# belacks/audio-denoising

Hardware: AMD Instinct MI355X
Metric: denoised audio frames/sec (32 ms, 16 kHz, hop 512) at batch 256; 1/2/4/8 GPU (higher is better)
Workload: dtype f32; 1 GPU; configs[1]: batch 256 synthetic 32 ms frames per GPU, n_fft=1024 hop=512 n_mels=80, GRUUNet2 fp32 (dari_tult weights, num_compressed_bins=5), 32-iter Griffin-Lim, device-RNG initial phases, hx carried; a step = one hop of 256 resident synthetic frames per GPU (the hops of a group are different frames; the same buffers are re-processed step after step: the path is compute-bound, no data-dependent w; streams_per_gpu=256, hops_per_launch=4, n_fft=1024, hop=512, n_mels=80, griffinlim_iters=32, conv_precision=fp32, parallelism=stream-sharded x1 (no data-path collective)

## Files before the change

audio-denoising_amd/csrc/dn_api.hip:

```cpp
#include <math.h>
#include <stdlib.h>
#include <string.h>

#include <atomic>
#include <thread>
#include <map>
#include <mutex>
#include <string>
#include <vector>

#include "dn_internal.hpp"

namespace {

thread_local std::string g_err;

int fail(int code, const std::string& msg) {
    g_err = msg;
    return code;
}

#define DN_HIP(call)                                                                                     \
    do {                                                                                                 \
        hipError_t e_ = (call);                                                                          \
// ... 853 lines not shown

size_t dn_clip_workspace_bytes(const dn_dsp* d, int32_t B, int32_t N) {
    if (!d || B <= 0 || N <= 0 || d->cfg.n_mels <= 0 || (long long)B * N > kClipMaxFrames) return 0;
    const size_t frames = (size_t)B * (size_t)N;
    return ((frames * (clip_row_floats(d) + 6 * (size_t)d->cfg.n_mels + 1) * sizeof(float) + 255) & ~size_t(255)) + 256;
}

size_t dn_clip_workspace_bytes_ex(const dn_dsp* d, int32_t B, int32_t N, uint32_t flags) {
    if (flags & ~(uint32_t)(DN_CONV_BF16 | DN_PHASE_FROM_INPUT | DN_CLIP_GL_PER_COLUMN | DN_CLIP_GL_PER_STREAM)) return 0;
    const size_t base = dn_clip_workspace_bytes(d, B, N);
    return base == 0 || !(flags & DN_PHASE_FROM_INPUT) ? base : base + phasor_bytes(d, (size_t)B * (size_t)N);
}

int dn_clip_process(const dn_model* m, const dn_dsp* d, const void* hops_in, int32_t in_s16, float* ring, float* ola, float* hx, void* hops_out,
                    int32_t out_s16, const float* init_angles, uint64_t seed, uint64_t stream_id0, int32_t n_iter, float momentum,
                    void* workspace, int32_t B, int32_t N, uint32_t flags, void* stream) {
    if (B < 1 || N < 1) return fail(DN_ERR_INVALID, "dn_clip_process: needs B >= 1 streams and N >= 1 hops");
    if (!hops_in || !ring || !ola || !hx || !hops_out || !workspace) return fail(DN_ERR_INVALID, "dn_clip_process: null argument");
    const uint32_t gl = flags & (uint32_t)(DN_CLIP_GL_PER_COLUMN | DN_CLIP_GL_PER_STREAM);
    int rc = check_hop_args("dn_clip_process", m, d, B, n_iter, momentum, flags & ~gl);
    if (rc != DN_OK) return rc;
    if (gl == (uint32_t)(DN_CLIP_GL_PER_COLUMN | DN_CLIP_GL_PER_STREAM))
        return fail(DN_ERR_INVALID, "dn_clip_process: DN_CLIP_GL_PER_COLUMN and DN_CLIP_GL_PER_STREAM exclude each other");
    if ((gl & DN_CLIP_GL_PER_STREAM) && d->cfg.n_fft != 1024)
        return fail(DN_ERR_UNSUPPORTED, "the wavefront-per-stream Griffin-Lim is built for n_fft 1024 (at 1536 the per-lane state of a stream does not fit a wavefront's registers; at 512 the schedule is not built)");
    if ((flags & DN_PHASE_FROM_INPUT) && init_angles) return fail(DN_ERR_INVALID, "dn_clip_process: DN_PHASE_FROM_INPUT takes the phases from the input: init_angles must be NULL");
    if ((long long)B * N > kClipMaxFrames)
        return fail(DN_ERR_INVALID, "dn_clip_process: B x N exceeds " + std::to_string(kClipMaxFrames) + " frames a call (tile the clip)");
    const int M = d->cfg.n_mels, C = M / 16;
    BiasSet* bs = nullptr;
    rc = build_bias(const_cast<dn_model*>(m), C, &bs);
    if (rc != DN_OK) return rc;
    dn::ClipArgs a{};
    a.hops_in = hops_in; a.in_s16 = in_s16 != 0; a.ring = ring; a.ola = ola; a.hx = hx; a.hops_out = hops_out; a.out_s16 = out_s16 != 0;
    a.init = init_angles; a.seed = seed; a.sid0 = stream_id0; a.n_iter = n_iter; a.mom = momentum / (1.0f + momentum);
    a.C = C; a.B = B; a.N = N; a.n_fft = d->cfg.n_fft; a.n_mels = M;
    a.frames = (size_t)B * (size_t)N;
    a.fr = static_cast<float*>(workspace); a.fr_stride = clip_row_floats(d);
    a.mel = a.fr + a.frames * a.fr_stride; a.diff = a.mel + a.frames * 3 * M; a.peak = a.diff + a.frames * 3 * M;
    if (flags & DN_PHASE_FROM_INPUT) a.phas = reinterpret_cast<float*>(static_cast<char*>(workspace) + dn_clip_workspace_bytes(d, B, N));
    a.per_stream = d->cfg.n_fft == 1024 && ((gl & DN_CLIP_GL_PER_STREAM) || (gl == 0 && (long)a.frames >= dn::kClipGlwAutoFrames));
    dn::launch_clip(d->view, bs->view_dev, a, (flags & DN_CONV_BF16) != 0, as_stream(stream));
    return check_launch("dn_clip_process");
}

static size_t slot_floats(const dn_dsp* d, int32_t B) {
    return (size_t)B * (6 * (size_t)d->cfg.n_mels + 1 + dn::kSlotMeta + 3 * ((size_t)d->cfg.n_fft / 2 + 1));
}

static int default_head_start(const dn_pipe* p) {
    return p->depth == 1 && p->B <= 256 ? (p->d->cfg.n_fft == 1536 ? 12 : 8) : 0;
}

int dn_pipe_create(const dn_model* m, const dn_dsp* d, int32_t B, uint32_t flags, dn_pipe** out) {
    if (!out) return fail(DN_ERR_INVALID, "dn_pipe_create: null argument");
    if (B <= 0) return fail(DN_ERR_INVALID, "dn_pipe_create: batch must be positive");
    int rc = check_hop_args("dn_pipe_create", m, d, B, 0, 0.0f, flags);
    if (rc != DN_OK) return rc;
    dn_pipe* p = new dn_pipe();
    p->m = const_cast<dn_model*>(m); p->d = const_cast<dn_dsp*>(d); p->B = B; p->C = d->cfg.n_mels / 16;
    p->bf16 = (flags & DN_CONV_BF16) != 0;
    p->phase_in = (flags & DN_PHASE_FROM_INPUT) != 0;
    p->m->refs.fetch_add(1);
    p->d->refs.fetch_add(1);
    rc = build_bias(p->m, p->C, &p->bs);
    if (rc != DN_OK) { dn_pipe_destroy(p); return rc; }
    p->slot_floats = (slot_floats(d, B) + 63) & ~size_t(63);
    p->init_elems = (size_t)B * 3 * (d->cfg.n_fft / 2 + 1);
    p->state_elems = (size_t)B * 3 * (2 * ((size_t)d->cfg.n_fft / 128) + 2) * 64;
    static_assert(sizeof(dn::PipeCtl) <= 256, "the control block fits its allocation");
    hipError_t e = hipMalloc(reinterpret_cast<void**>(&p->ctl), 256);
    if (e == hipSuccess) e = hipMemset(p->ctl, 0, 256);
    if (e == hipSuccess) e = hipMalloc(reinterpret_cast<void**>(&p->scratch), p->n_slots * p->slot_floats * sizeof(float));
    if (e == hipSuccess && p->phase_in) e = hipMalloc(reinterpret_cast<void**>(&p->scratch_init), p->n_slots * p->init_elems * sizeof(float2));
    if (e != hipSuccess) { dn_pipe_destroy(p); return fail(DN_ERR_HIP, std::string("dn_pipe_create: ") + hipGetErrorString(e)); }
    {
        const int it = default_head_start(p);
        if (it > 0) { rc = dn_pipe_set_head_start(p, it); if (rc != DN_OK) { dn_pipe_destroy(p); return rc; } }
    }
    *out = p;
    return DN_OK;
}

void dn_pipe_destroy(dn_pipe* p) {
    if (!p) return;
    if (p->hio) {
        HostIo* h = p->hio;
        if (h->h2d) (void)hipStreamSynchronize(h->h2d);
        if (h->d2h) (void)hipStreamSynchronize(h->d2h);
        for (int i = 0; i < HostIo::kRing; ++i) {
            if (h->ev_h2d[i]) (void)hipEventDestroy(h->ev_h2d[i]);
            if (h->ev_k[i]) (void)hipEventDestroy(h->ev_k[i]);
            if (h->ev_d2h[i]) (void)hipEventDestroy(h->ev_d2h[i]);
        }
        for (int i = 0; i < 2; ++i) {
            if (h->d_in[i]) (void)hipFree(h->d_in[i]);
            if (h->d_out[i]) (void)hipFree(h->d_out[i]);
            if (h->z_out[i]) (void)hipFree(h->z_out[i]);
        }
        if (h->h2d) (void)hipStreamDestroy(h->h2d);
        if (h->d2h) (void)hipStreamDestroy(h->d2h);
        if (h->done_host) (void)hipHostFree(h->done_host);
        delete h;
    }
    if (p->scratch) (void)hipFree(p->scratch);
    if (p->scratch_init) (void)hipFree(p->scratch_init);
    if (p->gl_state) (void)hipFree(p->gl_state);
    if (p->ctl) (void)hipFree(p->ctl);
    if (p->ring) (void)hipFree(p->ring);
    if (p->ola) (void)hipFree(p->ola);
    if (p->hx) (void)hipFree(p->hx);
    model_release(p->m);
    dsp_release(p->d);
    delete p;
}

int dn_pipe_set_head_start(dn_pipe* p, int32_t iterations) {
    if (!p || iterations < 0) return fail(DN_ERR_INVALID, "dn_pipe_set_head_start: bad argument");
    if (iterations > 0 && p->group > 0) return fail(DN_ERR_INVALID, "dn_pipe_set_head_start: a group pipe never parks a chain");
    if (iterations > 0 && p->split == DN_SPLIT_ON) return fail(DN_ERR_INVALID, "dn_pipe_set_head_start: the pipe splits every hop into two launches (dn_pipe_set_split(p, DN_SPLIT_OFF or DN_SPLIT_AUTO) first)");
    if (iterations > 0 && !p->gl_state) DN_HIP(hipMalloc(reinterpret_cast<void**>(&p->gl_state), p->n_slots * p->state_elems * sizeof(float2)));
    if (iterations > 0 && p->d->cfg.n_fft == 1536) {
        int rc = dn_pipe_reserve_parity(p);
        if (rc != DN_OK) return rc;
    }
    p->gl_split = iterations;
    return DN_OK;
}

int dn_pipe_set_depth(dn_pipe* p, int32_t depth) {
    if (!p) return fail(DN_ERR_INVALID, "dn_pipe_set_depth: null pipe");
    if (depth < 1 || depth > DN_PIPE_MAX_DEPTH) return fail(DN_ERR_INVALID, "dn_pipe_set_depth: depth must be in 1.." + std::to_string(DN_PIPE_MAX_DEPTH));
    if (depth > 1 && p->d->cfg.n_fft != 1024)
        return fail(DN_ERR_UNSUPPORTED, "pipes deeper than one hop are built for n_fft 1024 (at 1536 the per-lane state of a stream does not fit a wavefront's registers; at 512 the schedule is not built)");
    if (depth > 1 && p->group > 0) return fail(DN_ERR_INVALID, "dn_pipe_set_depth: a group pipe runs whole chains per launch (dn_pipe_set_group(p, 0) first)");
    if (depth == p->depth) return DN_OK;
    dn::PipeCtl h{};
    DN_HIP(hipDeviceSynchronize());
    DN_HIP(hipMemcpy(&h, p->ctl, sizeof(h), hipMemcpyDeviceToHost));
    if (h.pending != 0) return fail(DN_ERR_INVALID, "dn_pipe_set_depth: hops are in flight (flush first)");
    const int n_slots = depth + 1;
    float* scratch = nullptr;
    float2* state = nullptr;
    float2* init = nullptr;
    hipError_t e = hipMalloc(reinterpret_cast<void**>(&scratch), n_slots * p->slot_floats * sizeof(float));
    if (e == hipSuccess && depth > 1) e = hipMalloc(reinterpret_cast<void**>(&state), n_slots * p->state_elems * sizeof(float2));
    if (e == hipSuccess && (depth > 1 || p->phase_in)) e = hipMalloc(reinterpret_cast<void**>(&init), n_slots * p->init_elems * sizeof(float2));
    if (e != hipSuccess) {
        if (scratch) (void)hipFree(scratch);
        if (state) (void)hipFree(state);
        if (init) (void)hipFree(init);
        return fail(DN_ERR_HIP, std::string("dn_pipe_set_depth: ") + hipGetErrorString(e));
    }
    (void)hipFree(p->scratch);
    if (p->gl_state) (void)hipFree(p->gl_state);
    if (p->scratch_init) (void)hipFree(p->scratch_init);
    p->scratch = scratch; p->gl_state = state; p->scratch_init = init;
    p->depth = depth; p->n_slots = n_slots;
    p->gl_split = 0;
    h.slot_next = 0;
    DN_HIP(hipMemcpy(p->ctl, &h, sizeof(h), hipMemcpyHostToDevice));
    return dn_pipe_set_head_start(p, default_head_start(p));
}

int dn_pipe_set_group(dn_pipe* p, int32_t hops) {
    if (!p) return fail(DN_ERR_INVALID, "dn_pipe_set_group: null pipe");
    if (hops < 0 || hops > DN_PIPE_MAX_GROUP) return fail(DN_ERR_INVALID, "dn_pipe_set_group: hops must be in 0.." + std::to_string(DN_PIPE_MAX_GROUP));
    if (hops > 0 && p->d->cfg.n_fft != 1024)
        return fail(DN_ERR_UNSUPPORTED, "hop groups run whole Griffin-Lim chains one wavefront per stream, which is built for n_fft 1024 (at 1536 that form measured slower than a wavefront per column; at 512 it is not built)");
    if (hops > 0 && p->depth > 1) return fail(DN_ERR_INVALID, "dn_pipe_set_group: the pipe is deeper than one hop (dn_pipe_set_depth(p, 1) first)");
    if (hops > 0 && p->hio) return fail(DN_ERR_UNSUPPORTED, "dn_pipe_set_group: the host-buffer transport moves single hops");
    if (hops == p->group) return DN_OK;
    dn::PipeCtl h{};
    DN_HIP(hipDeviceSynchronize());
    DN_HIP(hipMemcpy(&h, p->ctl, sizeof(h), hipMemcpyDeviceToHost));
    if (h.pending != 0) return fail(DN_ERR_INVALID, "dn_pipe_set_group: hops are in flight (flush first)");
    const int n_slots = hops > 0 ? 2 * DN_PIPE_MAX_GROUP : p->depth + 1;
    float* scratch = nullptr;
    float2* init = nullptr;
    hipError_t e = hipMalloc(reinterpret_cast<void**>(&scratch), n_slots * p->slot_floats * sizeof(float));
    if (e == hipSuccess && p->scratch_init) e = hipMalloc(reinterpret_cast<void**>(&init), n_slots * p->init_elems * sizeof(float2));
    if (e != hipSuccess) {
        if (scratch) (void)hipFree(scratch);
        if (init) (void)hipFree(init);
        return fail(DN_ERR_HIP, std::string("dn_pipe_set_group: ") + hipGetErrorString(e));
    }
    (void)hipFree(p->scratch);
    if (p->scratch_init) (void)hipFree(p->scratch_init);
    if (p->gl_state) { (void)hipFree(p->gl_state); p->gl_state = nullptr; }
    p->scratch = scratch; p->scratch_init = init;
    p->n_slots = n_slots;
    p->group = hops; p->group_pending = 0;
    p->group_pushes = h.pushes;
    p->gl_split = 0;
    h.slot_next = 0;
    DN_HIP(hipMemcpy(p->ctl, &h, sizeof(h), hipMemcpyHostToDevice));
    return hops > 0 ? DN_OK : dn_pipe_set_head_start(p, default_head_start(p));
}

int dn_pipe_set_gl_schedule(dn_pipe* p, int32_t schedule) {
    if (!p) return fail(DN_ERR_INVALID, "dn_pipe_set_gl_schedule: null pipe");
    if (schedule != DN_GL_AUTO && schedule != DN_GL_WAVE_PER_COLUMN && schedule != DN_GL_WAVE_PER_STREAM)
        return fail(DN_ERR_INVALID, "dn_pipe_set_gl_schedule: unknown schedule");
    if (schedule == DN_GL_WAVE_PER_STREAM && p->d->cfg.n_fft != 1024)
        return fail(DN_ERR_UNSUPPORTED, "the wavefront-per-stream Griffin-Lim is built for n_fft 1024 (at 1536 the per-lane state of a stream does not fit a wavefront's registers; at 512 the schedule is not built)");
    if (schedule == DN_GL_WAVE_PER_COLUMN && p->depth > 1)
        return fail(DN_ERR_INVALID, "a pipe deeper than one hop runs a wavefront per stream and chain segment");
    if (schedule == DN_GL_WAVE_PER_COLUMN && p->group > 0)
        return fail(DN_ERR_INVALID, "a group pipe runs whole chains a wavefront per stream (dn_pipe_set_group(p, 0) first)");
    p->gl_schedule = schedule;
    return DN_OK;
}

int dn_pipe_set_split(dn_pipe* p, int32_t mode) {
    if (!p) return fail(DN_ERR_INVALID, "dn_pipe_set_split: null pipe");
    if (mode != DN_SPLIT_AUTO && mode != DN_SPLIT_OFF && mode != DN_SPLIT_ON) return fail(DN_ERR_INVALID, "dn_pipe_set_split: unknown mode");
    if (mode == DN_SPLIT_ON && p->d->cfg.n_fft != 1024)
        return fail(DN_ERR_UNSUPPORTED, "the split hop belongs to the wavefront-per-stream Griffin-Lim, which is built for n_fft 1024 (not for 512 or 1536)");
    if (mode == DN_SPLIT_ON && p->gl_split > 0)
        return fail(DN_ERR_INVALID, "dn_pipe_set_split: the pipe runs a head start (a front workgroup that goes on with its frame's chain cannot be a launch of its own): "
                                    "dn_pipe_set_head_start(p, 0) first");
    if (mode == DN_SPLIT_ON && p->group > 0) return fail(DN_ERR_INVALID, "dn_pipe_set_split: a group pipe is one launch per group");
    p->split = mode;
    return DN_OK;
}

int dn_pipe_set_model(dn_pipe* p, const dn_model* m) {
    if (!p || !m) return fail(DN_ERR_INVALID, "dn_pipe_set_model: null argument");
    if (m == p->m) return DN_OK;
    BiasSet* bs = nullptr;
    int rc = build_bias(const_cast<dn_model*>(m), p->C, &bs);
    if (rc != DN_OK) return rc;
    const_cast<dn_model*>(m)->refs.fetch_add(1);
    model_release(p->m);
    p->m = const_cast<dn_model*>(m);
    p->bs = bs;
    return DN_OK;
}

int dn_pipe_stream_create(const dn_model* m, const dn_dsp* d, int32_t B, uint32_t flags, dn_pipe** out) {
    dn_pipe* p = nullptr;
    int rc = dn_pipe_create(m, d, B, flags, &p);
    if (rc != DN_OK) return rc;
    const size_t line = (size_t)B * d->cfg.n_fft * sizeof(float), hxb = (size_t)B * dn::kHidden * p->C * sizeof(float);
    hipError_t e = hipMalloc(reinterpret_cast<void**>(&p->ring), line);
    if (e == hipSuccess) e = hipMalloc(reinterpret_cast<void**>(&p->ola), line);
    if (e == hipSuccess) e = hipMalloc(reinterpret_cast<void**>(&p->hx), hxb);
    if (e == hipSuccess) e = hipMemset(p->ring, 0, line);
    if (e == hipSuccess) e = hipMemset(p->ola, 0, line);
    if (e == hipSuccess) e = hipMemset(p->hx, 0, hxb);
// ... 22 lines not shown
    p->group_pushes = (unsigned long long)(p->d->cfg.n_fft / p->d->cfg.hop - 1);
    p->group_pending = 0;
    dn::launch_ctl_set(p->ctl, (unsigned long long)(p->d->cfg.n_fft / p->d->cfg.hop - 1), frames_done, 0, as_stream(stream));
    return check_launch("ctl_set_kernel");
}

int dn_pipe_get_counters(dn_pipe* p, uint64_t* pushes, uint64_t* frames, int32_t* pending, void* stream) {
    if (!p) return fail(DN_ERR_INVALID, "dn_pipe_get_counters: null pipe");
    dn::PipeCtl h{};
    DN_HIP(hipMemcpyAsync(&h, p->ctl, sizeof(h), hipMemcpyDeviceToHost, as_stream(stream)));
    DN_HIP(hipStreamSynchronize(as_stream(stream)));
    if (pushes) *pushes = h.pushes;
    if (frames) *frames = h.frames;
    if (pending) *pending = (int32_t)h.pending;
    return DN_OK;
}

int dn_pipe_reserve_parity(dn_pipe* p) {
    if (!p) return fail(DN_ERR_INVALID, "dn_pipe_reserve_parity: null pipe");
    if (!p->scratch_init) DN_HIP(hipMalloc(reinterpret_cast<void**>(&p->scratch_init), p->n_slots * p->init_elems * sizeof(float2)));
    return DN_OK;
}

static int fill_hop_args(dn_pipe* p, dn::HopArgs& a, const float* init_angles, uint64_t seed, uint64_t stream_id0, int32_t n_iter,
                         float momentum) {
    if (n_iter < 0) return fail(DN_ERR_INVALID, "negative n_iter");
    if (!(momentum >= 0.0f && momentum < 1.0f)) return fail(DN_ERR_INVALID, "momentum must be in [0, 1)");
    if (init_angles && p->phase_in) return fail(DN_ERR_INVALID, "this pipe was created with DN_PHASE_FROM_INPUT: it takes the phases from the input, init_angles must be NULL");
    if (init_angles && !p->scratch_init) {
        int rc = dn_pipe_reserve_parity(p);
        if (rc != DN_OK) return rc;
    }
    a.ctl = p->ctl;
    a.slots = p->scratch; a.slot_stride = p->slot_floats;
    a.slot_init = p->scratch_init; a.init_stride = p->init_elems;
    a.gl_state = p->gl_state; a.state_stride = p->state_elems;
    a.n_slots = p->n_slots;
    a.gl_split = p->gl_split;
    a.init_in = init_angles; a.seed = seed; a.sid0 = stream_id0;
    a.phase_in = p->phase_in ? 1 : 0;
    a.n_iter = n_iter; a.mom = momentum / (1.0f + momentum);
    a.B = p->B; a.C = p->C; a.back_B = p->B;
    const bool per_stream = p->depth > 1 || (p->d->cfg.n_fft == 1024 && (p->gl_schedule == DN_GL_WAVE_PER_STREAM ||
                                                                        (p->gl_schedule == DN_GL_AUTO && p->B >= dn::kGlwAutoStreams)));
    a.glw = per_stream ? 1 : 0;
    a.depth = p->depth;
    a.spb = per_stream ? 4 / p->depth : 1;
    a.back_blocks = (p->B + a.spb - 1) / a.spb;
    const bool can_split = per_stream && p->gl_split == 0;
    a.split = can_split && (p->split == DN_SPLIT_ON || (p->split == DN_SPLIT_AUTO && (long)p->B * p->depth >= dn::kSplitAutoChains)) ? 1 : 0;
    a.prime = p->d->cfg.n_fft / p->d->cfg.hop - 1;
    a.n_mels = p->d->cfg.n_mels; a.d_dev = p->d->view_dev; a.c_dev = p->bs->view_dev;
    if (p->group > 0) {
        a.glw = 1; a.depth = 1; a.split = 0; a.gl_split = 0;
        a.spb = p->group == 1 ? 4 : p->group == 2 ? 2 : 1;
        a.back_blocks = (p->B + a.spb - 1) / a.spb;
    }
    return DN_OK;
}

int dn_pipe_stream_push(dn_pipe* p, const void* hop_in, int32_t in_is_s16, void* hop_out, int32_t out_is_s16,
                        const float* init_angles, uint64_t seed, uint64_t stream_id0, int32_t n_iter, float momentum, void* stream) {
    if (!p || !p->ring) return fail(DN_ERR_INVALID, "dn_pipe_stream_push: not a streaming pipe");
    if (!hop_in || !hop_out) return fail(DN_ERR_INVALID, "dn_pipe_stream_push: null argument");
    if (p->group > 0) return fail(DN_ERR_INVALID, "dn_pipe_stream_push: this pipe takes groups of hops (dn_pipe_stream_push_group)");
    dn::HopArgs a{};
    int rc = fill_hop_args(p, a, init_angles, seed, stream_id0, n_iter, momentum);
    if (rc != DN_OK) return rc;
    a.front_B = p->B; a.hx = p->hx;
    a.host_done = p->host_done; a.host_done_value = p->host_done_value;
    a.host_copy_src = static_cast<const uint4*>(p->host_copy_src); a.host_copy_dst = static_cast<uint4*>(p->host_copy_dst);
    a.host_copy_n16 = (unsigned int)(p->host_copy_bytes / 16);
    a.hop_in = hop_in; a.ring = p->ring; a.in_s16 = in_is_s16;
    a.ola = p->ola; a.hop_out = hop_out; a.out_s16 = out_is_s16;
    dn::launch_hop(p->d->view, p->bs->view, a, p->bf16, as_stream(stream));
    rc = check_launch("hop_kernel(stream)");
    if (rc != DN_OK) return rc;
    ++p->group_pushes;
    return DN_OK;
}

static int host_io_init(dn_pipe* p) {
    if (p->hio) return DN_OK;
    HostIo* h = new HostIo();
    p->hio = h;
    const size_t bytes = (size_t)p->B * p->d->cfg.hop * sizeof(float);
    DN_HIP(hipStreamCreateWithFlags(&h->h2d, hipStreamNonBlocking));
    DN_HIP(hipStreamCreateWithFlags(&h->d2h, hipStreamNonBlocking));
    for (int i = 0; i < HostIo::kRing; ++i) {
        DN_HIP(hipEventCreateWithFlags(&h->ev_h2d[i], hipEventDisableTiming));
        DN_HIP(hipEventCreateWithFlags(&h->ev_k[i], hipEventDisableTiming));
        DN_HIP(hipEventCreateWithFlags(&h->ev_d2h[i], hipEventDisableTiming));
    }
    for (int i = 0; i < 2; ++i) {
        DN_HIP(hipMalloc(&h->d_in[i], bytes));
        DN_HIP(hipMalloc(&h->d_out[i], bytes));
    }
    DN_HIP(hipHostMalloc(reinterpret_cast<void**>(&h->done_host), 64, 0));
    *h->done_host = 0;
    void* dv = nullptr;
    DN_HIP(hipHostGetDevicePointer(&dv, h->done_host, 0));
    h->done_dev = static_cast<unsigned long long*>(dv);
    return DN_OK;
}

static void* device_view(const void* host) {
    hipPointerAttribute_t at;
// ... 563 lines not shown
```

audio-denoising_amd/csrc/dn_group.hip:

```cpp
#include "dn_hop_common.hpp"

namespace dn {

#ifdef DN_PROBE
static __device__ unsigned long long g_group_front[DN_PIPE_MAX_GROUP][4];
static __device__ unsigned long long g_group_wg[2048][2];
#define DN_GSTAMP(h, id) do { if (tid == 0 && (int)blockIdx.x == a.back_blocks) { unsigned long long t_; \
    asm volatile("s_memtime %0\n\ts_waitcnt lgkmcnt(0)" : "=s"(t_)::"memory"); g_group_front[h][id] = t_; } } while (0)
#define DN_GWG(id) do { if (tid == 0 && blockIdx.x < 2048) { unsigned long long t_; \
    asm volatile("s_memtime %0\n\ts_waitcnt lgkmcnt(0)" : "=s"(t_)::"memory"); g_group_wg[blockIdx.x][id] = t_; } } while (0)
#else
#define DN_GSTAMP(h, id) do { } while (0)
#define DN_GWG(id) do { } while (0)
#endif

template <int NFFT, bool STREAM, bool BF16, int CT, bool PHIN = false>
__global__ __launch_bounds__(kHopPipeThreads, 2) void group_kernel(DspDev d, const DspDev* __restrict__ dp, const CellDev* __restrict__ cp, HopArgs a) {
    static_assert(NFFT == 1024, "whole chains run one wavefront per stream beside a front wave (dn_glw_body.hpp): n_fft 1024");
    constexpr int kNR = NFFT, kBins = Geo<NFFT>::kBins, kHop = kNR / 2;
    constexpr int kPairs = kHop / 2, kFoldN = (kPairs + kHopPipeThreads - 1) / kHopPipeThreads;
    __shared__ __attribute__((aligned(16))) char smem[hop_smem<NFFT>()];
    const int tid = threadIdx.x;
    const unsigned long long pushes = a.ctl->pushes, frames = a.ctl->frames;
    const unsigned int pending = a.ctl->pending, slot_next = a.ctl->slot_next;
    const SlotLayout sl(a.B, a.n_mels, kBins);
    int prime_hops = 0;
    if (STREAM) {
        const long long left = (long long)a.prime - (long long)pushes;
        prime_hops = left <= 0 ? 0 : left < (long long)a.group_hops ? (int)left : a.group_hops;
    }
    const int fronted = a.front_B > 0 ? a.group_hops - prime_hops : 0;
    DN_GWG(0);
    if ((int)blockIdx.x < a.back_blocks) {
      {
        const int lane = tid & 63, wv = __builtin_amdgcn_readfirstlane(tid >> 6);
        const int per = kGlwWaves / a.spb, sidx = wv / per, j = wv - sidx * per;
        const size_t b = (size_t)blockIdx.x * a.spb + sidx;
        DN_WSTAMP(0);
        const bool runs = j < (int)pending && b < (size_t)a.back_B;
        if (pending && !runs) {
            glw_fill_tables<NFFT, kHopPipeThreads>(smem, d, tid);
            DN_LDS_BARRIER();
        }
        if (runs) {
            const int s = slot_behind(slot_next, (int)pending - j, a.n_slots);
            const float* slot = a.slots + (size_t)s * a.slot_stride;
            const uint32_t* meta = reinterpret_cast<const uint32_t*>(slot + sl.meta) + kSlotMeta * b;
            const v2f* init = meta[0] ? reinterpret_cast<const v2f*>(a.slot_init + (size_t)s * a.init_stride) : nullptr;
            const uint64_t seed = (uint64_t)meta[1] | ((uint64_t)meta[2] << 32);
            const uint64_t sid0 = (uint64_t)meta[3] | ((uint64_t)meta[4] << 32);
            const int n_iter = __builtin_amdgcn_readfirstlane((int)meta[6]);
            const float mom = __builtin_bit_cast(float, __builtin_amdgcn_readfirstlane((int)meta[7]));
            float* gl_out = reinterpret_cast<float*>((uint64_t)meta[8] | ((uint64_t)meta[9] << 32));
#ifdef DN_GLW_PRIO
            __builtin_amdgcn_s_setprio(DN_GLW_PRIO);
#endif
            glw_body<NFFT, STREAM ? kEmitStage : kEmitFrame>(smem, d, slot + sl.lin, init, seed, sid0, slot + sl.peak, gl_out, n_iter, mom, b, lane, wv,
                                                             nullptr, nullptr, 0, 0, -1, kGlwFresh, nullptr, tid);
            DN_WSTAMP(7);
        }
        if (STREAM) {
            __syncthreads();
            const int P = (int)pending;
            const int lead = a.filler_first ? a.group_out - P : 0;
            for (int si = 0; si < a.spb; ++si) {
                const size_t bs = (size_t)blockIdx.x * a.spb + si;
                if (bs >= (size_t)a.back_B) break;
                float* orow = a.ola + bs * kNR;
                v2f lo[kFoldN], hi[kFoldN];
#pragma unroll
                for (int r = 0; r < kFoldN; ++r) {
                    const int m = tid + kHopPipeThreads * r;
                    if (m < kPairs) { lo[r] = *reinterpret_cast<const v2f*>(orow + 2 * m); hi[r] = *reinterpret_cast<const v2f*>(orow + 2 * m + kHop); }
                }
                for (int i = 0; i < a.group_out; ++i) {
                    const int f = i - lead;
                    const bool has = f >= 0 && f < P;
                    const float* line = glw_signal_line<NFFT>(smem, si * per + (has ? f : 0));
                    const float sc = has ? (a.slots + (size_t)slot_behind(slot_next, P - f, a.n_slots) * a.slot_stride + sl.peak)[bs] : 0.0f;
#pragma unroll
                    for (int r = 0; r < kFoldN; ++r) {
                        const int m = tid + kHopPipeThreads * r;
                        if (m >= kPairs) continue;
                        v2f emit = mk2(0.0f, 0.0f);
                        if (has) {
                            emit = lo[r];
                            const v2f p0 = *reinterpret_cast<const v2f*>(line + 2 * m), p1 = *reinterpret_cast<const v2f*>(line + 2 * m + kHop);
                            lo[r] = mk2(fmaf(p0[0], sc, hi[r][0]), fmaf(p0[1], sc, hi[r][1]));
                            hi[r] = mk2(fmaf(p1[0], sc, 0.0f), fmaf(p1[1], sc, 0.0f));
                        }
                        const size_t at = (size_t)i * (size_t)a.hop_out_stride + bs * kHop + 2 * m;
                        if (a.out_s16) {
                            const float c0 = fminf(fmaxf(emit[0], -1.0f), 1.0f) * 32767.0f, c1 = fminf(fmaxf(emit[1], -1.0f), 1.0f) * 32767.0f;
                            *reinterpret_cast<unsigned int*>(static_cast<short*>(a.hop_out) + at) = (unsigned int)(unsigned short)(short)c0 | ((unsigned int)(unsigned short)(short)c1 << 16);
                        } else {
                            *reinterpret_cast<v2f*>(static_cast<float*>(a.hop_out) + at) = emit;
                        }
                    }
                }
                if (P > 0) {
#pragma unroll
                    for (int r = 0; r < kFoldN; ++r) {
                        const int m = tid + kHopPipeThreads * r;
                        if (m < kPairs) { *reinterpret_cast<v2f*>(orow + 2 * m) = lo[r]; *reinterpret_cast<v2f*>(orow + 2 * m + kHop) = hi[r]; }
                    }
                }
            }
        }
      }
    } else {
      {
        const size_t b = blockIdx.x - a.back_blocks;
#pragma unroll 1
        for (int h = 0; h < a.group_hops; ++h) {
            int z;
            DN_OPAQUE_ZERO(z);
            const DspDev& dz = dp[z];
            const CellDev& cz = cp[z];
            const int tidz = tid + z;
            const float* frames_in = STREAM ? a.ring : a.frames + (size_t)h * (size_t)a.frames_stride;
            if (STREAM) {
                const char* in = static_cast<const char*>(a.hop_in) + (size_t)h * (size_t)a.hop_in_stride * (a.in_s16 ? 2 : 4);
                ring_shift<NFFT, kHopPipeThreads>(a.ring, in, a.in_s16, b, tid);
            }
            if (h < prime_hops) continue;
            const int q = h - prime_hops;
            int s = (int)slot_next + q;
            if (s >= a.n_slots) s -= a.n_slots;
            float* slot = a.slots + (size_t)s * a.slot_stride;
            DN_GSTAMP(q, 0);
            stft_body<NFFT, false, true, kHopPipeThreads, PHIN>(smem, dz, frames_in, nullptr, slot, slot + sl.peak, DN_PEAK_NORMALIZE | DN_PRE_WINDOW, b, tidz,
                                                                PHIN ? a.slot_init + (size_t)s * a.init_stride : nullptr);
            __syncthreads();
            DN_GSTAMP(q, 1);
            cell_body<kHopPipeThreads / 64, BF16, CT>(smem, cz, slot, a.hx + z, slot + sl.diff, a.hx + z, 3, a.C, b, tidz);
            __syncthreads();
            DN_GSTAMP(q, 2);
            invmel_body<NFFT, true, kHopPipeThreads>(smem, dz, slot, slot + sl.diff, slot + sl.lin, 3 * a.B, b * 3, tidz);
            DN_GSTAMP(q, 3);
            if (tid == 0) {
                uint32_t* meta = reinterpret_cast<uint32_t*>(slot + sl.meta) + kSlotMeta * b;
                const uint64_t seed = a.seed + frames + (unsigned long long)q;
                meta[0] = (PHIN || a.init_in != nullptr) ? 1u : 0u;
                meta[1] = (uint32_t)seed;
                meta[2] = (uint32_t)(seed >> 32);
                meta[3] = (uint32_t)a.sid0;
                meta[4] = (uint32_t)(a.sid0 >> 32);
                meta[5] = 0u;
                meta[6] = (uint32_t)a.n_iter;
                meta[7] = __builtin_bit_cast(uint32_t, a.mom);
                const uint64_t dst = reinterpret_cast<uint64_t>(STREAM ? nullptr : a.gl_out + (size_t)h * (size_t)a.out_stride);
                meta[8] = (uint32_t)dst;
                meta[9] = (uint32_t)(dst >> 32);
            }
            if (!PHIN && a.init_in != nullptr) {
                const float2* src = reinterpret_cast<const float2*>(a.init_in + (size_t)h * (size_t)a.init_in_stride) + b * 3 * kBins;
                float2* dst = a.slot_init + (size_t)s * a.init_stride + b * 3 * kBins;
                for (int i = tid; i < 3 * kBins; i += kHopPipeThreads) dst[i] = src[i];
            }
            __syncthreads();
        }
      }
    }
    __syncthreads();
    DN_GWG(1);
    if (tid == 0) {
        const unsigned int t = atomicAdd(&a.ctl->done, 1u);
        if (t == gridDim.x - 1) {
            a.ctl->done = 0;
            a.ctl->launches = a.ctl->launches + 1;
            if (a.front_B > 0) a.ctl->pushes = pushes + (unsigned long long)a.group_hops;
            a.ctl->frames = frames + (unsigned long long)fronted;
            unsigned int sn = slot_next + (unsigned int)fronted;
            if (sn >= (unsigned int)a.n_slots) sn -= (unsigned int)a.n_slots;
            a.ctl->slot_next = sn;
            a.ctl->pending = (unsigned int)fronted;
        }
    }
}

void launch_group(const DspDev& d, const CellDev& c, const HopArgs& a, bool bf16, hipStream_t st) {
    const dim3 grid(a.back_blocks + a.front_B), block(kHopPipeThreads);
    const bool stream = a.ola != nullptr, usual = a.C == 5;
    auto go = [&](auto k) { hipLaunchKernelGGL(k, grid, block, 0, st, d, a.d_dev, a.c_dev, a); };
    auto pick = [&](auto stream_c, auto phin_c) {
        constexpr bool S = decltype(stream_c)::value, P = decltype(phin_c)::value;
        if (usual) { if (bf16) go(group_kernel<1024, S, true, 5, P>); else go(group_kernel<1024, S, false, 5, P>); }
        else { if (bf16) go(group_kernel<1024, S, true, 0, P>); else go(group_kernel<1024, S, false, 0, P>); }
    };
    using T = std::true_type; using F = std::false_type;
    const bool phin = a.phase_in && a.front_B > 0;
    if (stream) { if (phin) pick(T{}, T{}); else pick(T{}, F{}); }
    else { if (phin) pick(F{}, T{}); else pick(F{}, F{}); }
}

}

#ifdef DN_PROBE
extern "C" int dn_probe_read_group_glw(unsigned long long* host32) {
    return (int)hipMemcpyFromSymbol(host32, HIP_SYMBOL(dn::g_glw_probe), sizeof(dn::g_glw_probe));
}
extern "C" int dn_probe_read_group_front(unsigned long long* host16) {
    return (int)hipMemcpyFromSymbol(host16, HIP_SYMBOL(dn::g_group_front), sizeof(dn::g_group_front));
}
extern "C" int dn_probe_read_group_wg(unsigned long long* host4096) {
    return (int)hipMemcpyFromSymbol(host4096, HIP_SYMBOL(dn::g_group_wg), sizeof(dn::g_group_wg));
}
#endif
```

audio-denoising_amd/pipeline.py:

```python
from __future__ import annotations

import ctypes as C
import os

import torch

from . import _lib
from .gruunet2 import GRUUNet2
from .transforms import DspPlan, melscale_fbanks


class Denoiser:

    def __init__(self, model: GRUUNet2, sample_rate: int, n_fft: int = 1024, hop_length: int = 512, n_mels: int = 80,
                 n_iter: int = 32, momentum: float = 0.99, device=None, window: torch.Tensor | None = None, phase: str = "random"):
        self.device = torch.device(device if device is not None else next(model.parameters()).device)
        if self.device.type != "cuda":
            raise RuntimeError("Denoiser needs a 'cuda' device; there is no CPU path in this package")
        if phase not in ("random", "input"):
            raise ValueError("phase must be 'random' or 'input'")
        self.phase = phase
        if n_mels % 16 != 0:
            raise ValueError("n_mels must be a multiple of 16 (four stride-2 encoder levels)")
        self.lib = _lib.get_lib()
# ... 182 lines not shown
            st = C.c_void_p(torch.cuda.current_stream().cuda_stream)
            lib.check(lib.dn_stft_general(plan.handle, x.data_ptr(), spec.data_ptr(), logmel.data_ptr(), B, L, st))
            lib.check(lib.dn_cell_forward_ex(model_h, logmel.data_ptr(), hx0.data_ptr(), out.data_ptr(), hx1.data_ptr(), B, T, self.n_mels, Cb,
                                             self.hx_decay, st))
            lib.check(lib.dn_server_rows(plan.handle, logmel.data_ptr(), out.data_ptr(), spec.data_ptr(), spec.data_ptr(), B * T, st))
            lib.check(lib.dn_istft_general(plan.handle, spec.data_ptr(), wave.data_ptr(), B, T, st))
        return wave, hx1


class _Pipe:

    def __init__(self, denoiser: "Denoiser", batch: int, streaming: bool):
        import weakref
        self.dn, self.batch = denoiser, batch
        self.lib = denoiser.lib
        handle = C.c_void_p()
        self._owner = denoiser.model._native_owner(denoiser.device)
        self._flags = denoiser._flags()
        create = self.lib.dn_pipe_stream_create if streaming else self.lib.dn_pipe_create
        with torch.cuda.device(denoiser.device):
            self.lib.check(create(self._owner.handle, denoiser.plan.handle, batch, self._flags, C.byref(handle)))
        self.handle = handle
        self._fin = weakref.finalize(self, self.lib.dn_pipe_destroy, handle)
        hs = os.environ.get("DN_GL_HEAD_START")
        if hs is not None:
            self.lib.check(self.lib.dn_pipe_set_head_start(handle, int(hs)))
        self.depth = 1
        self.group = 0
        dp = os.environ.get("DN_PIPE_DEPTH")
        if dp is not None:
            self.set_depth(int(dp))
        sch = os.environ.get("DN_GL_SCHEDULE")
        if sch is not None:
            self.lib.check(self.lib.dn_pipe_set_gl_schedule(handle, int(sch)))

        sp = os.environ.get("DN_PIPE_SPLIT")
        if sp is not None:
            self.set_split(int(sp))

    def set_split(self, mode: int) -> None:
        self.lib.check(self.lib.dn_pipe_set_split(self.handle, int(mode)))

    def set_gl_schedule(self, schedule: int) -> None:
        self.lib.check(self.lib.dn_pipe_set_gl_schedule(self.handle, int(schedule)))

    def set_depth(self, depth: int) -> None:
        with torch.cuda.device(self.dn.device):
            self.lib.check(self.lib.dn_pipe_set_depth(self.handle, int(depth)))
        self.depth = int(depth)

    def set_group(self, hops: int) -> None:
        with torch.cuda.device(self.dn.device):
            self.lib.check(self.lib.dn_pipe_set_group(self.handle, int(hops)))
        self.group = int(hops)

    def set_head_start(self, iterations: int) -> None:
        self.lib.check(self.lib.dn_pipe_set_head_start(self.handle, int(iterations)))

    def _bind(self) -> None:
        owner = self.dn.model._native_owner(self.dn.device)
        if owner is not self._owner:
            self.lib.check(self.lib.dn_pipe_set_model(self.handle, owner.handle))
            self._owner = owner
        if self.dn._flags() != self._flags:
            raise RuntimeError("conv_precision changed after the pipeline was created; create a new pipeline")

    def counters(self):
        a, b, c = C.c_uint64(), C.c_uint64(), C.c_int32()
        with torch.cuda.device(self.dn.device):
            st = C.c_void_p(torch.cuda.current_stream().cuda_stream)
            self.lib.check(self.lib.dn_pipe_get_counters(self.handle, C.byref(a), C.byref(b), C.byref(c), st))
        return a.value, b.value, bool(c.value)


class HopPipeline(_Pipe):

    def __init__(self, denoiser: "Denoiser", batch: int):
        super().__init__(denoiser, batch, streaming=False)

    def submit(self, frames: torch.Tensor, hx: torch.Tensor, out: torch.Tensor, seed: int = 0, stream_id0: int = 0,
               init_angles: torch.Tensor | None = None, check_weights: bool = True) -> None:
        d = self.dn
        if check_weights:
            self._bind()
        keep, ia_ptr = d._angles_ptr(init_angles, self.batch)
        with torch.cuda.device(d.device):
            st = C.c_void_p(torch.cuda.current_stream().cuda_stream)
            self.lib.check(self.lib.dn_pipe_submit(self.handle, frames.data_ptr(), hx.data_ptr(), out.data_ptr(), ia_ptr, seed, stream_id0,
                                                   d.n_iter, d.momentum, st))
            if keep is not None and not torch.cuda.is_current_stream_capturing():
                keep.record_stream(torch.cuda.current_stream())

    def submit_group(self, frames: torch.Tensor, hx: torch.Tensor, out: torch.Tensor, seed: int = 0, stream_id0: int = 0,
                     init_angles: torch.Tensor | None = None, check_weights: bool = True) -> None:
        d = self.dn
        if frames.dim() != 3 or tuple(out.shape) != tuple(frames.shape) or frames.shape[1:] != (self.batch, d.n_fft):
            raise ValueError(f"frames and out must both be (H, {self.batch}, {d.n_fft})")
        for t in (frames, out):
            if t.dtype != torch.float32 or t.device != d.device or t.stride(2) != 1 or t.stride(1) != d.n_fft:
                raise ValueError("frames and out must be float32 on the denoiser's device with contiguous (B, n_fft) hops")
        H = frames.shape[0]
        if check_weights:
            self._bind()
        ia_ptr, ia_stride, keep = None, 0, []
        if init_angles is not None:
            if init_angles.shape[0] != H:
# ... 397 lines not shown
```

Baseline: 7.059 million frames/s.

## Give group pipes a Griffin-Lim head start in front blocks after producing hops

Group pipes may now use a head start. After running STFT, cell and inverse-mel for its group of hops, each front block immediately runs the first few Griffin-Lim iterations of each fresh hop, one wavefront per hop, and saves the state to gl_state. The back blocks then resume from that saved segment in the next launch. The default for groups of three or more hops is one iteration, meant to fill idle wavefronts in the front blocks and shorten the back-block critical path. In exchange it adds a state save and reload, a larger gl_state allocation, and control-flow restructuring that may raise register pressure.

```diff
diff --git a/audio-denoising_amd/csrc/dn_api.hip b/audio-denoising_amd/csrc/dn_api.hip
--- a/audio-denoising_amd/csrc/dn_api.hip
+++ b/audio-denoising_amd/csrc/dn_api.hip
@@ -929,6 +929,11 @@
     return p->depth == 1 && p->B <= 256 ? (p->d->cfg.n_fft == 1536 ? 12 : 8) : 0;
 }
 
+static int default_group_head_start(const dn_pipe* p) {
+    constexpr int kGroupHeadStart = 1;
+    return p->group >= 3 && p->B <= 256 ? kGroupHeadStart : 0;
+}
+
 int dn_pipe_create(const dn_model* m, const dn_dsp* d, int32_t B, uint32_t flags, dn_pipe** out) {
     if (!out) return fail(DN_ERR_INVALID, "dn_pipe_create: null argument");
     if (B <= 0) return fail(DN_ERR_INVALID, "dn_pipe_create: batch must be positive");
@@ -994,7 +999,6 @@
 
 int dn_pipe_set_head_start(dn_pipe* p, int32_t iterations) {
     if (!p || iterations < 0) return fail(DN_ERR_INVALID, "dn_pipe_set_head_start: bad argument");
-    if (iterations > 0 && p->group > 0) return fail(DN_ERR_INVALID, "dn_pipe_set_head_start: a group pipe never parks a chain");
     if (iterations > 0 && p->split == DN_SPLIT_ON) return fail(DN_ERR_INVALID, "dn_pipe_set_head_start: the pipe splits every hop into two launches (dn_pipe_set_split(p, DN_SPLIT_OFF or DN_SPLIT_AUTO) first)");
     if (iterations > 0 && !p->gl_state) DN_HIP(hipMalloc(reinterpret_cast<void**>(&p->gl_state), p->n_slots * p->state_elems * sizeof(float2)));
     if (iterations > 0 && p->d->cfg.n_fft == 1536) {
@@ -1072,7 +1076,7 @@
     p->gl_split = 0;
     h.slot_next = 0;
     DN_HIP(hipMemcpy(p->ctl, &h, sizeof(h), hipMemcpyHostToDevice));
-    return hops > 0 ? DN_OK : dn_pipe_set_head_start(p, default_head_start(p));
+    return dn_pipe_set_head_start(p, hops > 0 ? default_group_head_start(p) : default_head_start(p));
 }
 
 int dn_pipe_set_gl_schedule(dn_pipe* p, int32_t schedule) {
@@ -1201,7 +1205,7 @@
     a.prime = p->d->cfg.n_fft / p->d->cfg.hop - 1;
     a.n_mels = p->d->cfg.n_mels; a.d_dev = p->d->view_dev; a.c_dev = p->bs->view_dev;
     if (p->group > 0) {
-        a.glw = 1; a.depth = 1; a.split = 0; a.gl_split = 0;
+        a.glw = 1; a.depth = 1; a.split = 0;
         a.spb = p->group == 1 ? 4 : p->group == 2 ? 2 : 1;
         a.back_blocks = (p->B + a.spb - 1) / a.spb;
     }
diff --git a/audio-denoising_amd/csrc/dn_group.hip b/audio-denoising_amd/csrc/dn_group.hip
--- a/audio-denoising_amd/csrc/dn_group.hip
+++ b/audio-denoising_amd/csrc/dn_group.hip
@@ -5,6 +5,9 @@
 #ifdef DN_PROBE
 static __device__ unsigned long long g_group_front[DN_PIPE_MAX_GROUP][4];
 static __device__ unsigned long long g_group_wg[2048][2];
+static __device__ unsigned long long g_group_hs[kGlwWaves][2];
+#define DN_GHS(id) do { if ((int)blockIdx.x == a.back_blocks && (tid & 63) == 0) { unsigned long long t_; \
+    asm volatile("s_memtime %0\n\ts_waitcnt lgkmcnt(0)" : "=s"(t_)::"memory"); g_group_hs[tid >> 6][id] = t_; } } while (0)
 #define DN_GSTAMP(h, id) do { if (tid == 0 && (int)blockIdx.x == a.back_blocks) { unsigned long long t_; \
     asm volatile("s_memtime %0\n\ts_waitcnt lgkmcnt(0)" : "=s"(t_)::"memory"); g_group_front[h][id] = t_; } } while (0)
 #define DN_GWG(id) do { if (tid == 0 && blockIdx.x < 2048) { unsigned long long t_; \
@@ -12,6 +15,7 @@
 #else
 #define DN_GSTAMP(h, id) do { } while (0)
 #define DN_GWG(id) do { } while (0)
+#define DN_GHS(id) do { } while (0)
 #endif
 
 template <int NFFT, bool STREAM, bool BF16, int CT, bool PHIN = false>
@@ -30,35 +34,132 @@
         prime_hops = left <= 0 ? 0 : left < (long long)a.group_hops ? (int)left : a.group_hops;
     }
     const int fronted = a.front_B > 0 ? a.group_hops - prime_hops : 0;
+    const bool back = (int)blockIdx.x < a.back_blocks;
     DN_GWG(0);
-    if ((int)blockIdx.x < a.back_blocks) {
-      {
-        const int lane = tid & 63, wv = __builtin_amdgcn_readfirstlane(tid >> 6);
+    bool runs = false, fills = false;
+    size_t gb = 0;
+    const float* gslot = nullptr;
+    const v2f* ginit = nullptr;
+    v2f* gstate = nullptr;
+    float* gout = nullptr;
+    uint64_t gseed = 0, gsid0 = 0;
+    int g_n_iter = 0, g_begin = 0, g_stop = -1, g_resume = kGlwFresh, gwv = 0;
+    float gmom = 0.0f;
+    if (back) {
+        const int wv = __builtin_amdgcn_readfirstlane(tid >> 6);
         const int per = kGlwWaves / a.spb, sidx = wv / per, j = wv - sidx * per;
-        const size_t b = (size_t)blockIdx.x * a.spb + sidx;
+        gb = (size_t)blockIdx.x * a.spb + sidx;
+        gwv = wv;
         DN_WSTAMP(0);
-        const bool runs = j < (int)pending && b < (size_t)a.back_B;
-        if (pending && !runs) {
-            glw_fill_tables<NFFT, kHopPipeThreads>(smem, d, tid);
-            DN_LDS_BARRIER();
-        }
+        runs = j < (int)pending && gb < (size_t)a.back_B;
+        fills = pending && !runs;
         if (runs) {
             const int s = slot_behind(slot_next, (int)pending - j, a.n_slots);
-            const float* slot = a.slots + (size_t)s * a.slot_stride;
-            const uint32_t* meta = reinterpret_cast<const uint32_t*>(slot + sl.meta) + kSlotMeta * b;
-            const v2f* init = meta[0] ? reinterpret_cast<const v2f*>(a.slot_init + (size_t)s * a.init_stride) : nullptr;
-            const uint64_t seed = (uint64_t)meta[1] | ((uint64_t)meta[2] << 32);
-            const uint64_t sid0 = (uint64_t)meta[3] | ((uint64_t)meta[4] << 32);
-            const int n_iter = __builtin_amdgcn_readfirstlane((int)meta[6]);
-            const float mom = __builtin_bit_cast(float, __builtin_amdgcn_readfirstlane((int)meta[7]));
-            float* gl_out = reinterpret_cast<float*>((uint64_t)meta[8] | ((uint64_t)meta[9] << 32));
+            gslot = a.slots + (size_t)s * a.slot_stride;
+            const uint32_t* meta = reinterpret_cast<const uint32_t*>(gslot + sl.meta) + kSlotMeta * gb;
+            ginit = meta[0] ? reinterpret_cast<const v2f*>(a.slot_init + (size_t)s * a.init_stride) : nullptr;
+            gseed = (uint64_t)meta[1] | ((uint64_t)meta[2] << 32);
+            gsid0 = (uint64_t)meta[3] | ((uint64_t)meta[4] << 32);
+            g_begin = __builtin_amdgcn_readfirstlane((int)meta[5]);
+            g_n_iter = __builtin_amdgcn_readfirstlane((int)meta[6]);
+            gmom = __builtin_bit_cast(float, __builtin_amdgcn_readfirstlane((int)meta[7]));
+            gout = reinterpret_cast<float*>((uint64_t)meta[8] | ((uint64_t)meta[9] << 32));
+            g_resume = g_begin > 0 ? kGlwFromSeg : kGlwFresh;
+            gstate = a.gl_state != nullptr ? reinterpret_cast<v2f*>(a.gl_state + (size_t)s * a.state_stride) : nullptr;
 #ifdef DN_GLW_PRIO
             __builtin_amdgcn_s_setprio(DN_GLW_PRIO);
 #endif
-            glw_body<NFFT, STREAM ? kEmitStage : kEmitFrame>(smem, d, slot + sl.lin, init, seed, sid0, slot + sl.peak, gl_out, n_iter, mom, b, lane, wv,
-                                                             nullptr, nullptr, 0, 0, -1, kGlwFresh, nullptr, tid);
-            DN_WSTAMP(7);
-        }
+        }
+    } else {
+      {
+        const size_t b = blockIdx.x - a.back_blocks;
+#pragma unroll 1
+        for (int h = 0; h < a.group_hops; ++h) {
+            int z;
+            DN_OPAQUE_ZERO(z);
+            const DspDev& dz = dp[z];
+            const CellDev& cz = cp[z];
+            const int tidz = tid + z;
+            const float* frames_in = STREAM ? a.ring : a.frames + (size_t)h * (size_t)a.frames_stride;
+            if (STREAM) {
+                const char* in = static_cast<const char*>(a.hop_in) + (size_t)h * (size_t)a.hop_in_stride * (a.in_s16 ? 2 : 4);
+                ring_shift<NFFT, kHopPipeThreads>(a.ring, in, a.in_s16, b, tid);
+            }
+            if (h < prime_hops) continue;
+            const int q = h - prime_hops;
+            int s = (int)slot_next + q;
+            if (s >= a.n_slots) s -= a.n_slots;
+            float* slot = a.slots + (size_t)s * a.slot_stride;
+            DN_GSTAMP(q, 0);
+            stft_body<NFFT, false, true, kHopPipeThreads, PHIN>(smem, dz, frames_in, nullptr, slot, slot + sl.peak, DN_PEAK_NORMALIZE | DN_PRE_WINDOW, b, tidz,
+                                                                PHIN ? a.slot_init + (size_t)s * a.init_stride : nullptr);
+            __syncthreads();
+            DN_GSTAMP(q, 1);
+            cell_body<kHopPipeThreads / 64, BF16, CT>(smem, cz, slot, a.hx + z, slot + sl.diff, a.hx + z, 3, a.C, b, tidz);
+            __syncthreads();
+            DN_GSTAMP(q, 2);
+            invmel_body<NFFT, true, kHopPipeThreads>(smem, dz, slot, slot + sl.diff, slot + sl.lin, 3 * a.B, b * 3, tidz);
+            DN_GSTAMP(q, 3);
+            if (tid == 0) {
+                uint32_t* meta = reinterpret_cast<uint32_t*>(slot + sl.meta) + kSlotMeta * b;
+                const uint64_t seed = a.seed + frames + (unsigned long long)q;
+                meta[0] = (PHIN || a.init_in != nullptr) ? 1u : 0u;
+                meta[1] = (uint32_t)seed;
+                meta[2] = (uint32_t)(seed >> 32);
+                meta[3] = (uint32_t)a.sid0;
+                meta[4] = (uint32_t)(a.sid0 >> 32);
+                meta[5] = (uint32_t)min(a.gl_split, a.n_iter);
+                meta[6] = (uint32_t)a.n_iter;
+                meta[7] = __builtin_bit_cast(uint32_t, a.mom);
+                const uint64_t dst = reinterpret_cast<uint64_t>(STREAM ? nullptr : a.gl_out + (size_t)h * (size_t)a.out_stride);
+                meta[8] = (uint32_t)dst;
+                meta[9] = (uint32_t)(dst >> 32);
+            }
+            if (!PHIN && a.init_in != nullptr) {
+                const float2* src = reinterpret_cast<const float2*>(a.init_in + (size_t)h * (size_t)a.init_in_stride) + b * 3 * kBins;
+                float2* dst = a.slot_init + (size_t)s * a.init_stride + b * 3 * kBins;
+                for (int i = tid; i < 3 * kBins; i += kHopPipeThreads) dst[i] = src[i];
+            }
+            __syncthreads();
+        }
+        const int split = fronted > 0 ? min(a.gl_split, a.n_iter) : 0;
+        if (split > 0) {
+            const int wv = __builtin_amdgcn_readfirstlane(tid >> 6);
+            gwv = wv;
+            runs = wv < fronted;
+            fills = !runs;
+            if (runs) {
+                int s = (int)slot_next + wv;
+                if (s >= a.n_slots) s -= a.n_slots;
+                gb = b;
+                gslot = a.slots + (size_t)s * a.slot_stride;
+                ginit = (PHIN || a.init_in != nullptr) ? reinterpret_cast<const v2f*>(a.slot_init + (size_t)s * a.init_stride) : nullptr;
+                gseed = a.seed + frames + (unsigned long long)wv;
+                gsid0 = a.sid0;
+                g_n_iter = a.n_iter;
+                gmom = a.mom;
+                g_stop = split;
+                gstate = reinterpret_cast<v2f*>(a.gl_state + (size_t)s * a.state_stride);
+#ifdef DN_GHS_PRIO
+                __builtin_amdgcn_s_setprio(DN_GHS_PRIO);
+#endif
+            }
+            DN_GHS(0);
+        }
+      }
+    }
+    if (fills) {
+        glw_fill_tables<NFFT, kHopPipeThreads>(smem, d, tid);
+        DN_LDS_BARRIER();
+    }
+    if (runs) {
+        glw_body<NFFT, STREAM ? kEmitStage : kEmitFrame>(smem, d, gslot + sl.lin, ginit, gseed, gsid0, gslot + sl.peak, gout, g_n_iter, gmom, gb, tid & 63, gwv,
+                                                         nullptr, nullptr, 0, g_begin, g_stop, g_resume, gstate, tid);
+        if (back) DN_WSTAMP(7); else DN_GHS(1);
+    }
+    if (back) {
+      {
+        const int per = kGlwWaves / a.spb;
         if (STREAM) {
             __syncthreads();
             const int P = (int)pending;
@@ -108,59 +209,6 @@
             }
         }
       }
-    } else {
-      {
-        const size_t b = blockIdx.x - a.back_blocks;
-#pragma unroll 1
-        for (int h = 0; h < a.group_hops; ++h) {
-            int z;
-            DN_OPAQUE_ZERO(z);
-            const DspDev& dz = dp[z];
-            const CellDev& cz = cp[z];
-            const int tidz = tid + z;
-            const float* frames_in = STREAM ? a.ring : a.frames + (size_t)h * (size_t)a.frames_stride;
-            if (STREAM) {
-                const char* in = static_cast<const char*>(a.hop_in) + (size_t)h * (size_t)a.hop_in_stride * (a.in_s16 ? 2 : 4);
-                ring_shift<NFFT, kHopPipeThreads>(a.ring, in, a.in_s16, b, tid);
-            }
-            if (h < prime_hops) continue;
-            const int q = h - prime_hops;
-            int s = (int)slot_next + q;
-            if (s >= a.n_slots) s -= a.n_slots;
-            float* slot = a.slots + (size_t)s * a.slot_stride;
-            DN_GSTAMP(q, 0);
-            stft_body<NFFT, false, true, kHopPipeThreads, PHIN>(smem, dz, frames_in, nullptr, slot, slot + sl.peak, DN_PEAK_NORMALIZE | DN_PRE_WINDOW, b, tidz,
-                                                                PHIN ? a.slot_init + (size_t)s * a.init_stride : nullptr);
-            __syncthreads();
-            DN_GSTAMP(q, 1);
-            cell_body<kHopPipeThreads / 64, BF16, CT>(smem, cz, slot, a.hx + z, slot + sl.diff, a.hx + z, 3, a.C, b, tidz);
-            __syncthreads();
-            DN_GSTAMP(q, 2);
-            invmel_body<NFFT, true, kHopPipeThreads>(smem, dz, slot, slot + sl.diff, slot + sl.lin, 3 * a.B, b * 3, tidz);
-            DN_GSTAMP(q, 3);
-            if (tid == 0) {
-                uint32_t* meta = reinterpret_cast<uint32_t*>(slot + sl.meta) + kSlotMeta * b;
-                const uint64_t seed = a.seed + frames + (unsigned long long)q;
-                meta[0] = (PHIN || a.init_in != nullptr) ? 1u : 0u;
-                meta[1] = (uint32_t)seed;
-                meta[2] = (uint32_t)(seed >> 32);
-                meta[3] = (uint32_t)a.sid0;
-                meta[4] = (uint32_t)(a.sid0 >> 32);
-                meta[5] = 0u;
-                meta[6] = (uint32_t)a.n_iter;
-                meta[7] = __builtin_bit_cast(uint32_t, a.mom);
-                const uint64_t dst = reinterpret_cast<uint64_t>(STREAM ? nullptr : a.gl_out + (size_t)h * (size_t)a.out_stride);
-                meta[8] = (uint32_t)dst;
-                meta[9] = (uint32_t)(dst >> 32);
-            }
-            if (!PHIN && a.init_in != nullptr) {
-                const float2* src = reinterpret_cast<const float2*>(a.init_in + (size_t)h * (size_t)a.init_in_stride) + b * 3 * kBins;
-                float2* dst = a.slot_init + (size_t)s * a.init_stride + b * 3 * kBins;
-                for (int i = tid; i < 3 * kBins; i += kHopPipeThreads) dst[i] = src[i];
-            }
-            __syncthreads();
-        }
-      }
     }
     __syncthreads();
     DN_GWG(1);
@@ -203,6 +251,9 @@
 extern "C" int dn_probe_read_group_front(unsigned long long* host16) {
     return (int)hipMemcpyFromSymbol(host16, HIP_SYMBOL(dn::g_group_front), sizeof(dn::g_group_front));
 }
+extern "C" int dn_probe_read_group_hs(unsigned long long* host8) {
+    return (int)hipMemcpyFromSymbol(host8, HIP_SYMBOL(dn::g_group_hs), sizeof(dn::g_group_hs));
+}
 extern "C" int dn_probe_read_group_wg(unsigned long long* host4096) {
     return (int)hipMemcpyFromSymbol(host4096, HIP_SYMBOL(dn::g_group_wg), sizeof(dn::g_group_wg));
 }
diff --git a/audio-denoising_amd/pipeline.py b/audio-denoising_amd/pipeline.py
--- a/audio-denoising_amd/pipeline.py
+++ b/audio-denoising_amd/pipeline.py
@@ -258,6 +258,9 @@
     def set_group(self, hops: int) -> None:
         with torch.cuda.device(self.dn.device):
             self.lib.check(self.lib.dn_pipe_set_group(self.handle, int(hops)))
+            hs = os.environ.get("DN_GL_HEAD_START")
+            if hs is not None:
+                self.lib.check(self.lib.dn_pipe_set_head_start(self.handle, int(hs)))
         self.group = int(hops)
 
     def set_head_start(self, iterations: int) -> None:
```

Result: no change. 7.099 million frames/s (median of 6 runs) (+0.6%).
